# zhangzhousuper/Radish_PT

Hardware: AMD Instinct MI355X
Metric: Mrays/s (higher is better)
Workload: dtype f32

## Files before the change

radish_pt_amd/csrc/device/kernels_wave.h:

```cpp
#pragma once
#include "kernels_pt.h"
#include "wg_trace.h"
#include "ray_cull.h"
#include "kernels_walk.h"

namespace rd {

constexpr int kWfLitCap = 8192;
constexpr int kWfLitShadow = 0x40000000;
constexpr int kMaxWaveDepth = 32;

struct alignas(128) WaveCounter {
    int v;
    int pad[31];
};
#ifndef RD_WF_TICKET_SHARDS
#define RD_WF_TICKET_SHARDS 8
#endif
constexpr int kTicketShards = RD_WF_TICKET_SHARDS;
struct WaveCounters {
    WaveCounter rayCount[kMaxWaveDepth + 2];
    WaveCounter shadowCount[kMaxWaveDepth + 2];
    WaveCounter litCount[kMaxWaveDepth + 2];
    WaveCounter litShadowCount[kMaxWaveDepth + 2];
    WaveCounter traceHead[kMaxWaveDepth + 2];
    WaveCounter shadeHead[kMaxWaveDepth + 2][4];
    WaveCounter traceTicket[kMaxWaveDepth + 2][kTicketShards];
    WaveCounter shadeTicket[kMaxWaveDepth + 2][kTicketShards];
};

struct WaveWorkspace {
    float4 *ro[2];
    float4 *rd[2];
    float4 *thr[2];
    float4 *prevPos[2];
    float4 *accD;
    float4 *accI;
    float4 *nee[2];
    float4 *sht[2];
    uint2 *rng[2];
    int4 *hit;
    int *rayq[2];
    int *shadowq;
    int *litq[2];
    int litCap;
    int *treeOvf;
    int treeOvfDepth;
#ifdef RD_WF_STAMPS
    unsigned long long *stamps;
    int stampWaves;
    int stampStages;
#endif
    WaveCounters *ctr;
};

constexpr unsigned kWfNeeNone = 2u;
RD_DEV float wfNeeTag(int home, unsigned kind) { return __uint_as_float(((unsigned)home << 2) | kind); }
RD_DEV void wfAddNee(const WaveWorkspace &w, float4 n) {
    const unsigned tag = __float_as_uint(n.w), kind = tag & 3u;
    if (kind == kWfNeeNone) return;
    float4 *acc = (kind == 0u ? w.accD : w.accI) + (tag >> 2);
    const float4 a = *acc;
    *acc = make_float4(a.x + n.x, a.y + n.y, a.z + n.z, 0.f);
}

RD_DEV Ray wfSlotRay(const WaveWorkspace &w, int set, int p, bool shadow, float &limit) {
    if (shadow) {
        const float4 x = w.prevPos[set][p], y = w.sht[set][p];
        return shadowRay(mk3(x.x, x.y, x.z), mk3(y.x, y.y, y.z), limit);
    }
    const float4 o = w.ro[set][p], d = w.rd[set][p];
    limit = 3.402823466e+38f;
    return Ray{mk3(o.x, o.y, o.z), mk3(d.x, d.y, d.z)};
}

struct WaveSlotPath {
    const WaveWorkspace &w;
    const int rs, p;
    const int wr, q;
    int home;
    const bool delta;
    bool nullNee = false;
    RD_DEV v3 throughput() {
        const float4 t = w.thr[rs][p];
        home = __float_as_int(t.w);
        return mk3(t.x, t.y, t.z);
    }
    RD_DEV float samplePdf() const { return w.ro[rs][p].w; }
    RD_DEV bool sampleDelta() const { return delta; }
    RD_DEV v3 prevPos() const { const float4 c = w.prevPos[rs][p]; return mk3(c.x, c.y, c.z); }
    RD_DEV void setDirect(v3 v) { w.accD[home] = make_float4(v.x, v.y, v.z, 0.f); }
    RD_DEV void addIndirect(v3 v) { const float4 a = w.accI[home]; w.accI[home] = make_float4(a.x + v.x, a.y + v.y, a.z + v.z, 0.f); }
    RD_DEV Sampler rng(const DScene &s) const { const uint2 r = w.rng[rs][p]; return Sampler{s.sobol, r.x, (int)r.y}; }
    RD_DEV void setNee(v3 c, float nw) {
        w.nee[wr][q] = make_float4(c.x, c.y, c.z, wfNeeTag(home, nw < 0.f ? kWfNeeNone : (nw == 0.f ? 0u : 1u)));
        nullNee = nw < 0.f || (c.x == 0.f && c.y == 0.f && c.z == 0.f);
    }
    RD_DEV void setPrevPos(v3 x) { w.prevPos[wr][q] = make_float4(x.x, x.y, x.z, 0.f); }
    RD_DEV void setRay(const Ray &ray, float pdf, bool deltaSample, v3 throughput, const Sampler &rng) {
        w.ro[wr][q] = make_float4(ray.o.x, ray.o.y, ray.o.z, pdf);
        w.rd[wr][q] = make_float4(ray.d.x, ray.d.y, ray.d.z, deltaSample ? 1.f : 0.f);
        w.thr[wr][q] = make_float4(throughput.x, throughput.y, throughput.z, __int_as_float(home));
        w.rng[wr][q] = make_uint2(rng.scramble, (unsigned)rng.ptr);
    }
};


RD_DEV void waveAppend(bool pred, int item, int *queue, int *count) {
    unsigned long long mask = __ballot(pred);
    if (mask == 0ull) return;
    int leader = __ffsll((long long)mask) - 1;
    int base = 0;
    if ((int)(threadIdx.x & 63u) == leader) base = atomicAdd(count, __popcll(mask));
    base = __shfl(base, leader, 64);
    if (pred) queue[base + __popcll(mask & laneMaskLt())] = item;
}

constexpr int kShadeChunks = 4;
constexpr int kShadePacket = 64 * kShadeChunks;
#ifndef RD_WF_APPEND_CHUNKS
#define RD_WF_APPEND_CHUNKS 16
#endif
static_assert(RD_WF_APPEND_CHUNKS == 4 || RD_WF_APPEND_CHUNKS == 8 || RD_WF_APPEND_CHUNKS == 16, "RD_WF_APPEND_CHUNKS: 4, 8 or 16");
constexpr int kAppendSpan = 64 * RD_WF_APPEND_CHUNKS;

constexpr int kPacket = 128;
RD_DEV int gridWaves() { return int(gridDim.x * (blockDim.x >> 6)); }
RD_DEV int workgroupTicket(WaveCounter *tickets) {
    __shared__ int ticket;
    if (threadIdx.x == 0) {
        const unsigned x = blockIdx.x % (unsigned)kTicketShards;
        ticket = int(x + (unsigned)kTicketShards * (unsigned)atomicAdd(&tickets[x].v, 1));
    }
    __syncthreads();
    return __builtin_amdgcn_readfirstlane(ticket);
}
RD_DEV int logicalWave(int wg) { return __builtin_amdgcn_readfirstlane(int(wg * int(blockDim.x >> 6) + int(threadIdx.x >> 6))); }
RD_DEV int wavePull(int *head, int packet) {
    int base = 0;
    if ((threadIdx.x & 63u) == 0u) base = atomicAdd(head, packet);
    return __shfl(base, 0, 64) + gridWaves() * packet;
}
RD_DEV int tracePull(int *head, int headBase) {
    int base = 0;
    if ((threadIdx.x & 63u) == 0u) base = atomicAdd(head, kPacket);
    return __builtin_amdgcn_readlane(base, 0) + headBase;
}

RD_DEV unsigned subFrameBlocks(const PixelMap &pm, int part, int parts) { return (unsigned)(pm.numBlocks - part + parts - 1) / (unsigned)parts; }
constexpr int kSobolRows = 10000;
template <bool LENS>
RD_DEV void wfRaygen(const DScene &s, const DCamera &cam, const PixelMap &pm, const WaveWorkspace &w, int looper, int samples, int part,
                     int parts, const DLens &lens) {
    unsigned wg;
    const unsigned nLocal = subFrameBlocks(pm, part, parts);
    const unsigned nGroups = nLocal * (unsigned)samples;
    bool wgValid = xcdSwizzle(blockIdx.x, (nGroups + 3u) >> 2, wg);
    unsigned lane = threadIdx.x & 63u;
    unsigned group = wgValid ? wg * 4u + (threadIdx.x >> 6) : 0xffffffffu / 64u;
    const bool inRange = wgValid && group < nGroups;
    const unsigned b = group / nLocal, blockLocal = group - b * nLocal;
    Pix px = mapPixel(pm, inRange ? blockLocal * (unsigned)parts + (unsigned)part : 0xffffffffu / 64u, lane);
    bool valid = px.valid && inRange;
    int p = int(group * 64u + lane);
    bool listed = false;
    if (valid) {
        Sampler rng = makeSeededRandomEngine(int(((unsigned)looper + b) % (unsigned)kSobolRows), px.index, 0, s.sobol);
        Ray ray = cameraSample<LENS>(cam, px.x, px.y, sample4D(rng), lens);
        w.ro[0][p] = make_float4(ray.o.x, ray.o.y, ray.o.z, 0.f);
        w.rd[0][p] = make_float4(ray.d.x, ray.d.y, ray.d.z, 0.f);
        w.accD[p] = make_float4(0.f, 0.f, 0.f, 0.f);
        w.accI[p] = make_float4(0.f, 0.f, 0.f, 0.f);
        w.rng[0][p] = make_uint2(rng.scramble, (unsigned)rng.ptr);
        if (fabs_(ray.d.x) < 1.1e-6f || fabs_(ray.d.y) < 1.1e-6f || fabs_(ray.d.z) < 1.1e-6f) {
            const int at = atomicAdd(&w.ctr->litCount[0].v, 1);
            if (at < w.litCap) {
                w.litq[0][at] = p;
                listed = true;
            }
        }
    }
    if (inRange) w.rayq[0][p] = valid ? (listed ? -2 - p : p) : -1;
    if (blockIdx.x == 0 && threadIdx.x == 0) w.ctr->rayCount[0].v = int(nGroups) * 64;
}
__global__ __launch_bounds__(256) void k_wf_raygen(DScene s, DCamera cam, PixelMap pm, WaveWorkspace w, int looper, int samples, int part,
                                                   int parts) {
    wfRaygen<false>(s, cam, pm, w, looper, samples, part, parts, DLens{});
}
__global__ __launch_bounds__(256) void k_wf_raygen_lens(DScene s, DCamera cam, PixelMap pm, WaveWorkspace w, int looper, int samples,
                                                        int part, int parts, DLens lens) {
    wfRaygen<true>(s, cam, pm, w, looper, samples, part, parts, lens);
}

#ifndef RD_WF_DUTY_SHARE
#define RD_WF_DUTY_SHARE 0
#endif
#ifndef RD_REFILL_MIN
#define RD_REFILL_MIN 16
#endif
#ifndef RD_WF_FINISH_MIN
#define RD_WF_FINISH_MIN 16
#endif
#ifndef RD_WF_SHADOW_FIRST
#define RD_WF_SHADOW_FIRST 0
#endif
constexpr int kWfStampKinds = 6;
#ifdef RD_WF_STAMPS
#define RD_WF_STAMP(kind) do { if (stampAt && (threadIdx.x & 63u) == 0u) stampAt[kind] = wall_clock64(); } while (0)
#define RD_WF_STAMP_DRY() do { if (exhausted && !stampedDry) { stampedDry = true; RD_WF_STAMP(1); if (stampAt && (threadIdx.x & 63u) == 0u) *headDry = 1ull; } } while (0)
#define RD_WF_STAMP_HELD(held) do { if (stampAt && !stampedHeld && *headDry != 0ull) { \
        stampedHeld = true; const int h_ = (held); if ((threadIdx.x & 63u) == 0u) stampAt[4] = 1ull + (unsigned long long)h_; } } while (0)
#else
#define RD_WF_STAMP(kind) ((void)0)
#define RD_WF_STAMP_DRY() ((void)0)
#define RD_WF_STAMP_HELD(held) ((void)0)
#endif
#ifndef RD_WF_COOP_LONE
#define RD_WF_COOP_LONE 1
#endif

#ifndef RD_WF_TRACE_WAVES
#define RD_WF_TRACE_WAVES 7
#endif
#ifndef RD_WF_PAIR_WAVES
#define RD_WF_PAIR_WAVES 1
#endif
#ifndef RD_WF_PAIR_MAX_WAVES
#define RD_WF_PAIR_MAX_WAVES 6
#endif
template <bool COUNT, bool PAIRS = false>
__global__ __launch_bounds__(256) __attribute__((amdgpu_waves_per_eu(PAIRS && !COUNT ? RD_WF_PAIR_WAVES : (!COUNT ? RD_WF_TRACE_WAVES : 1),
                                                                      PAIRS && !COUNT ? RD_WF_PAIR_MAX_WAVES : 8))) void k_wf_trace(DScene s, WaveWorkspace w, int k) {
    WaveCounters *c = w.ctr;
    const int wg = workgroupTicket(c->traceTicket[k]);
#ifdef RD_WF_STAMPS
    unsigned long long *const stampAt = w.stamps ? w.stamps + ((size_t)k * (size_t)w.stampWaves + (size_t)logicalWave(wg)) * kWfStampKinds : nullptr;
    volatile unsigned long long *const headDry = w.stamps ? w.stamps + (size_t)w.stampStages * (size_t)w.stampWaves * kWfStampKinds + k : nullptr;
    bool stampedDry = false, stampedHeld = false;
    RD_WF_STAMP(0);
#endif
    const int nShadow = (k > 0) ? c->shadowCount[k - 1].v : 0;
    const int nRay = c->rayCount[k].v;
    const int total = nShadow + nRay;
    const int *rayq = w.rayq[k & 1];
    const int set = k & 1;
    WalkStats ws{0, 0};
    unsigned nClosest = 0, nAny = 0, nHits = 0;
    const int end = s.bvhSize;
    const int END = end;

    const int nLit = c->litCount[k].v < w.litCap ? c->litCount[k].v : w.litCap;
    const int dutyGroups = RD_WF_DUTY_SHARE ? 0 : (nLit < int(gridDim.x) ? nLit : int(gridDim.x));
    const bool duty = wg < dutyGroups;
    const int headBase = (int(gridDim.x) - dutyGroups) * int(blockDim.x >> 6) * kPacket;
    int resNext = duty ? headBase : (logicalWave(wg) - dutyGroups * int(blockDim.x >> 6)) * kPacket, resEnd = duty ? resNext : resNext + kPacket;
    bool exhausted = resNext >= total;
    if (resEnd > total) resEnd = total;
    RD_WF_STAMP_DRY();

    bool alive = false;
    bool isShadow = false;
    int p = -1;
    RaySlab rs;
    rs.o = rs.d = rs.inv = mk3(0.f);
    rs.cls = 0;
    const NodeRec *nodes = s.nodes[0];
    int ord = 0, cur = kPairNone;
    PairStack sp{0, 0};
    int node = END, pending = -1;
    float tmax = 0.f;
    int hitPrim = -1;
    v2 hitBary = mk2(0.f, 0.f);
    bool occluded = false;

    constexpr int kStackEntries = PAIRS ? 4 * kPairLds * 64 : 1;
    __shared__ union WfTraceLds {
        WgTraceSharedT<256> wg;
        int2 stack[kStackEntries];
    } lds;
    WgTraceSharedT<256> &wgsh = lds.wg;
    int2 *const stk = lds.stack + (PAIRS ? int(threadIdx.x >> 6) * kPairLds * 64 : 0);
    int2 *const ovf = PAIRS ? reinterpret_cast<int2 *>(w.treeOvf) + (size_t)logicalWave(wg) * (size_t)w.treeOvfDepth * 64 : nullptr;
    for (int it = wg; it < nLit; it += int(gridDim.x)) {
        const int e = w.litq[k & 1][it];
        const bool sh = (e & kWfLitShadow) != 0;
        const int pp = e & (kWfLitShadow - 1);
        float lim;
        const Ray ray = wfSlotRay(w, set, pp, sh, lim);
        const RaySlab urs = makeRaySlab(ray);
        if (urs.cls == 0 || end == 0) continue;
        const NodeRec *un = s.nodes[getMTBVHId(-ray.d)];
        const CoopTrace ct = sh ? wgTraceWhole<true, 256>(s, un, urs, lim, wgsh) : wgTraceWhole<false, 256>(s, un, urs, lim, wgsh);
        if (threadIdx.x == 0) {
            if (sh) {
                nAny++;
                if (!ct.found) wfAddNee(w, w.nee[set][pp]);
            } else {
                nClosest++;
                const bool hit = ct.hitPrim != -1;
                if (hit) nHits++;
                w.hit[pp] = make_int4(ct.hitPrim, __float_as_int(hit ? ct.bary.x : 0.f), __float_as_int(hit ? ct.bary.y : 0.f),
                                      hit ? int(s.primClass[ct.hitPrim]) : 0);
            }
            if (COUNT) {
                ws.nodes += ct.nodes;
                ws.tris += ct.tris;
            }
        }
    }
    RD_WF_STAMP(3);
#ifdef RD_WF_STAMPS
    if (stampAt && (threadIdx.x & 63u) == 0u) stampAt[5] = 1ull + (unsigned long long)nLit;
#endif
    if (PAIRS) __syncthreads();
    bool firstRound = true;
    bool fromList = false;
    for (;;) {
        bool doStart = false;
        fromList = false;
        if (firstRound) {
            firstRound = false;
            const int it = wg + (int(threadIdx.x & 63u) * 4 + int(threadIdx.x >> 6)) * int(gridDim.x);
            if (it < nLit) {
                const int e = w.litq[k & 1][it];
                doStart = true;
                fromList = true;
                isShadow = (e & kWfLitShadow) != 0;
                p = e & (kWfLitShadow - 1);
            }
        }
        unsigned long long idle = __ballot(!alive && !doStart && p < 0);
        int nIdle = __popcll(idle);
        if (!exhausted && nIdle >= RD_REFILL_MIN) {
            RD_WF_STAMP_HELD(resEnd - resNext);
            int myRank = __popcll(idle & laneMaskLt());
            int taken = 0;
            while (taken < nIdle && !exhausted) {
                if (resNext == resEnd) {
                    resNext = tracePull(&c->traceHead[k].v, headBase);
                    resEnd = resNext + kPacket;
                    if (resNext >= total) {
                        exhausted = true;
                        break;
                    }
                    if (resEnd > total) resEnd = total;
                }
                int avail = resEnd - resNext;
                int give = (nIdle - taken) < avail ? (nIdle - taken) : avail;
                if (!alive && !doStart && p < 0 && myRank >= taken && myRank < taken + give) {
                    const int item = resNext + (myRank - taken);
                    doStart = true;
#if RD_WF_SHADOW_FIRST
                    isShadow = item < nShadow;
                    p = isShadow ? w.shadowq[item] : rayq[item - nShadow];
#else
                    isShadow = item >= nRay;
                    p = isShadow ? w.shadowq[item - nRay] : rayq[item];
#endif
                }
                resNext += give;
                taken += give;
            }
        }
        RD_WF_STAMP_DRY();
        if (doStart) {
            if (p >= 0) {
                const Ray ray = wfSlotRay(w, set, p, isShadow, tmax);
                if (isShadow) nAny++;
                else nClosest++;
                rs = makeRaySlab(ray);
                pending = -1;
                if (PAIRS) {
                    ord = getMTBVHId(-ray.d);
                    sp = PairStack{0, 0};
                    if (rs.cls == 0 || end == 0) pairStart<COUNT>(s, rs, tmax, cur, pending, ws);
                    else cur = kPairFresh;
                    alive = true;
                } else {
                    nodes = s.nodes[getMTBVHId(-ray.d)];
                    node = 0;
                    alive = node != END;
                }
                hitPrim = -1;
                occluded = false;
                if (fromList && rs.cls != 0 && end != 0) {
                    if (isShadow) nAny--;
                    else nClosest--;
                    alive = false;
                    p = -1;
                }
            }
        }
        unsigned long long am = __ballot(alive);
        if (am == 0ull) {
            if (exhausted) break;
            continue;
        }

        {
            unsigned long long lit = __ballot(PAIRS ? (alive && cur == kPairFresh) : (alive && rs.cls != 0 && node == 0 && pending < 0));
            while (lit) {
                const int L = __ffsll((long long)lit) - 1;
                lit &= lit - 1ull;
                const bool shadowL = readlaneI(isShadow ? 1 : 0, L) != 0;
                const NodeRec *un = PAIRS ? s.nodes[0] + (size_t)readlaneI(ord, L) * (size_t)(end + 1) : readlanePtr(nodes, L);
                const RaySlab ur = readlaneRay(rs, L);
                const float lim = readlaneF(tmax, L);
                CoopTrace ct = shadowL ? coopTraceWhole<true>(s, un, ur, lim) : coopTraceWhole<false>(s, un, ur, lim);
                if (int(threadIdx.x & 63u) == L) {
                    hitPrim = ct.hitPrim;
                    hitBary = ct.bary;
                    tmax = ct.tmax;
                    occluded = ct.found;
                    node = END;
                    cur = kPairNone;
                    alive = false;
                    if (COUNT) {
                        ws.nodes += ct.nodes;
                        ws.tris += ct.tris;
                    }
                }
            }
        }
        if (PAIRS) {
            bool busy = alive && pending < 0;
            const int nStart = __popcll(__ballot(busy));
            if (nStart > 0) {
                const int minWalk = (nStart * (RD_LEAF_DEN - RD_LEAF_NUM) + RD_LEAF_DEN - 1) / RD_LEAF_DEN;
                const int lane = int(threadIdx.x & 63u);
                do {
                    pairPopOne<COUNT>(stk, lane, ovf, tmax, busy, cur, sp, pending, ws);
                    if (busy && cur >= 0) {
                        pairStep<COUNT>(s.pairs, stk, lane, ovf, rs, tmax, ord, cur, sp, pending, ws);
                        busy = pending < 0 && (cur >= 0 || sp.sp > 0);
                    }
                } while (__popcll(__ballot(busy)) >= (minWalk > 1 ? minWalk : 1));
                alive = alive && (pending >= 0 || cur >= 0 || sp.sp > 0);
            }
        } else
        {
            bool walking = alive && pending < 0;
            const int nStart = __popcll(__ballot(walking));
#if RD_WF_COOP_LONE
            if (nStart == 1) {
                const int L = __ffsll((long long)__ballot(walking)) - 1;
                CoopResult cr = coopWalk(readlanePtr(nodes, L), readlaneI(node, L), end, readlaneRay(rs, L), readlaneF(tmax, L), RD_COOP_WINDOWS);
                if (int(threadIdx.x & 63u) == L) {
                    node = cr.node;
                    pending = cr.pending;
                    if (COUNT) ws.nodes += cr.visited;
                    alive = (node != end) || pending >= 0;
                }
            } else
#endif
            if (nStart > 0) {
                const int minWalk = (nStart * (RD_LEAF_DEN - RD_LEAF_NUM) + RD_LEAF_DEN - 1) / RD_LEAF_DEN;
                do {
                    if (walking) {
                        if (COUNT) ws.nodes++;
                        float4 lo = nodes[node].lo_prim;
                        float4 hi = nodes[node].hi_next;
                        float boundDist;
                        bool boundHit = aabbFast(lo, hi, rs, boundDist);
                        if (boundHit && boundDist < tmax) {
                            pending = __float_as_int(lo.w);
                            node++;
                        } else {
                            node = __float_as_int(hi.w);
                        }
                        walking = pending < 0 && node != END;
                        alive = (node != END) || pending >= 0;
                    }
                } while (__popcll(__ballot(walking)) >= (minWalk > 1 ? minWalk : 1));
            }
        }
        if (alive && pending >= 0) {
            TriVerts t = loadTri(s.tris, pending);
            float dist;
            v2 bary;
            if (COUNT) ws.tris++;
            bool hit = intersectTriangle(rs, t.a, t.b, t.c, bary, dist);
            if (hit && dist < tmax) {
                if (isShadow) {
                    occluded = true;
                    node = END;
                    cur = kPairNone;
                    sp = PairStack{0, 0};
                } else {
                    hitPrim = pending;
                    tmax = dist;
                    hitBary = bary;
                }
            }
            pending = -1;
            alive = PAIRS ? (cur >= 0 || sp.sp > 0) : (node != END);
        }
        const unsigned long long doneM = __ballot(!alive && p >= 0);
        if (doneM != 0ull && __popcll(doneM) * 64 >= (__popcll(doneM) + __popcll(__ballot(alive))) * RD_WF_FINISH_MIN)
        if (!alive && p >= 0) {
            if (isShadow) {
                if (!occluded) wfAddNee(w, w.nee[set][p]);
            } else {
                bool hit = hitPrim != -1;
                if (hit) nHits++;
                w.hit[p] = make_int4(hitPrim, __float_as_int(hit ? hitBary.x : 0.f), __float_as_int(hit ? hitBary.y : 0.f),
                                     hit ? int(s.primClass[hitPrim]) : 0);
            }
            p = -1;
        }
    }
    RD_WF_STAMP(2);
    if (COUNT) flushCounters(s.counters, nClosest, nAny, nHits, ws);
}

struct WfSlotWork {
    const WaveWorkspace &w;
    int p;

    RD_DEV bool find(long long chunk, int slot) {
        const int e = w.rayq[0][chunk * 64 + slot];
        p = e <= -2 ? -2 - e : e;
        return e != -1;
    }
    RD_DEV Ray ray(float &tmax) const { return wfSlotRay(w, 0, p, false, tmax); }
    RD_DEV void store(const DScene &s, const RaySlab &, int hitPrim, v2 hitBary, float, bool) const {
        const bool hit = hitPrim != -1;
        w.hit[p] = make_int4(hitPrim, __float_as_int(hit ? hitBary.x : 0.f), __float_as_int(hit ? hitBary.y : 0.f),
                             hit ? int(s.primClass[hitPrim]) : 0);
    }
};
#ifndef RD_WF_PRIMARY_WAVES
#define RD_WF_PRIMARY_WAVES 1
#endif
template <bool COUNT>
__global__ __launch_bounds__(256, COUNT ? 1 : RD_WF_PRIMARY_WAVES) void k_wf_trace_primary(DScene s, WaveWorkspace w, int nGroups, int budget) {
    __shared__ WgTraceSharedT<256> wgsh;
    const int nLit = w.ctr->litCount[0].v < w.litCap ? w.ctr->litCount[0].v : w.litCap;
    WalkStats ws{0, 0};
    unsigned nClosest = 0, nHits = 0;
    for (int it = int(blockIdx.x); it < nLit; it += int(gridDim.x)) {
        const int pp = w.litq[0][it];
        float lim;
        const Ray ray = wfSlotRay(w, 0, pp, false, lim);
        const RaySlab urs = makeRaySlab(ray);
        if (!raySetAside(urs.cls) || s.bvhSize == 0) continue;
        const CoopTrace ct = wgTraceWhole<false, 256>(s, s.nodes[getMTBVHId(-ray.d)], urs, lim, wgsh);
        if (threadIdx.x == 0) {
            nClosest++;
            const bool hit = ct.hitPrim != -1;
            if (hit) nHits++;
            w.hit[pp] = make_int4(ct.hitPrim, __float_as_int(hit ? ct.bary.x : 0.f), __float_as_int(hit ? ct.bary.y : 0.f),
                                  hit ? int(s.primClass[ct.hitPrim]) : 0);
            if (COUNT) {
                ws.nodes += ct.nodes;
                ws.tris += ct.tris;
            }
        }
    }
    if (COUNT && threadIdx.x < 64u) flushCounters(s.counters, nClosest, 0u, nHits, ws);
    const int group = int(blockIdx.x) * 4 + int(threadIdx.x >> 6);
    if (group >= nGroups) return;
    const bool listed = w.rayq[0][(size_t)group * 64 + (threadIdx.x & 63u)] <= -2;
    WfSlotWork work{w, -1};
    walkPacket<COUNT, true>(s, group, listed, budget, work);
}

constexpr int kSortChunks = 16;
constexpr int kSortPacket = 64 * kSortChunks;
#ifndef RD_WF_SHADE_WAVES
#define RD_WF_SHADE_WAVES 1
#endif
#ifndef RD_WF_CULL_LAST
#define RD_WF_CULL_LAST 1
#endif
#ifndef RD_WF_SKIP_NULL_NEE
#define RD_WF_SKIP_NULL_NEE 1
#endif
__global__ __launch_bounds__(256, RD_WF_SHADE_WAVES) void k_wf_shade(DScene s, WaveWorkspace w, int k, int maxDepth, int sorted,
                                                                     const float4 *__restrict__ emitBox, int walkAll) {
    __shared__ int sSorted[4][kSortPacket];
    WaveCounters *c = w.ctr;
    const bool cullLast = RD_WF_CULL_LAST && !walkAll && k + 1 == maxDepth && !hasEnvMap(s);
    const bool skipNull = RD_WF_SKIP_NULL_NEE && !walkAll;
    float4 boxLo = make_float4(0.f, 0.f, 0.f, 0.f), boxHi = boxLo;
    if (cullLast) {
        boxLo = emitBox[0];
        boxHi = emitBox[1];
    }
    const int wg = workgroupTicket(c->shadeTicket[k]);
    const int lane = int(threadIdx.x & 63u);
    int *mySorted = sSorted[threadIdx.x >> 6];
    {
        const int q = 0;
        const int n = c->rayCount[k].v;
        const int *hitq = w.rayq[k & 1];
        int pendShadows = 0, pendRays = 0;
        int packet = kShadePacket;
        if (sorted) {
            const int perWave = n / (2 * gridWaves());
            packet = ((perWave + kShadePacket - 1) / kShadePacket) * kShadePacket;
            packet = packet < kShadePacket ? kShadePacket : (packet > kSortPacket ? kSortPacket : packet);
        }
        int packetEnd = 0;
        for (int base = logicalWave(wg) * packet, sub = 0, fresh = 1;;) {
            if (sub == packet) {
                base = wavePull(&c->shadeHead[k][q].v, packet);
                sub = 0;
                fresh = 1;
            }
            if (base + sub >= n) break;
            if (sorted && fresh) {
                fresh = 0;
                packetEnd = (n - base) < packet ? (n - base) : packet;
                int pp[kSortChunks], cls[kSortChunks];
#pragma unroll
                for (int j = 0; j < kSortChunks; j++) {
                    const int i = base + j * 64 + lane;
                    pp[j] = (j * 64 + lane < packetEnd) ? hitq[i] : -1;
                    if (pp[j] <= -2) pp[j] = -2 - pp[j];
                }
#pragma unroll
                for (int j = 0; j < kSortChunks; j++) {
                    cls[j] = (pp[j] >= 0) ? w.hit[pp[j]].w : 0;
                }
                int at = 0;
#pragma unroll
                for (int qq = 0; qq < 4; qq++) {
#pragma unroll
                    for (int j = 0; j < kSortChunks; j++) {
                        const bool in = (j * 64 + lane < packetEnd) && cls[j] == qq;
                        const unsigned long long m = __ballot(in);
                        if (in) mySorted[at + __popcll(m & laneMaskLt())] = pp[j];
                        at += __popcll(m);
                    }
                }
                __builtin_amdgcn_wave_barrier();
            }
            int item = base + sub + lane;
            const int subNow = sub;
            sub += 64;
            bool active = sorted ? (subNow + lane < packetEnd) : (item < n);
            bool emitShadow = false, emitRay = false, litShadow = false, litRay = false, rayFirst = false;
            int p = -1;
            const int q = base + subNow + lane;
            if (active) {
                p = sorted ? mySorted[subNow + lane] : hitq[item];
                if (p <= -2) p = -2 - p;
                active = p >= 0;
            }
            if (active) {
                const int4 h = w.hit[p];
                const float4 rdw = w.rd[k & 1][p];
                WaveSlotPath st{w, k & 1, p, (k + 1) & 1, q, p, rdw.w != 0.f};
                const PathStepResult r = pathStep(s, k, maxDepth, h.x, mk2(__int_as_float(h.y), __int_as_float(h.z)), mk3(rdw.x, rdw.y, rdw.z), st);
                if (r.shadow && !(skipNull && st.nullNee)) {
                    w.sht[(k + 1) & 1][q] = make_float4(r.shadowTo.x, r.shadowTo.y, r.shadowTo.z, 0.f);
                    emitShadow = true;
                    const v3 dl = r.shadowTo - r.shadowFrom;
                    const float l2 = dot(dl, dl) * 1.21e-12f;
                    litShadow = dl.x * dl.x < l2 || dl.y * dl.y < l2 || dl.z * dl.z < l2;
                }
                if (r.extension && !(cullLast && !mayReachEmitters(boxLo, boxHi, r.ray.o, r.ray.d))) {
                    emitRay = true;
                    litRay = fabs_(r.ray.d.x) < 1.1e-6f || fabs_(r.ray.d.y) < 1.1e-6f || fabs_(r.ray.d.z) < 1.1e-6f;
                }
            }
            if (__ballot(litShadow || litRay) != 0ull) {
                int *lq = w.litq[(k + 1) & 1];
                int *lc = &c->litCount[k + 1].v;
                for (int kind = 0; kind < 2; kind++) {
                    const bool pred = kind == 0 ? litShadow : litRay;
                    const unsigned long long m = __ballot(pred);
                    if (m == 0ull) continue;
                    int at = 0;
                    if (lane == 0) at = atomicAdd(lc, __popcll(m));
                    at = __shfl(at, 0, 64) + __popcll(m & laneMaskLt());
                    if (kind == 0) {
                        const int listed = __popcll(__ballot(pred && at < w.litCap));
                        if (lane == 0 && listed > 0) atomicAdd(&c->litShadowCount[k].v, listed);
                    }
                    if (pred && at < w.litCap) {
                        lq[at] = kind == 0 ? (q | kWfLitShadow) : q;
                        if (kind == 0) emitShadow = false;
                        else rayFirst = true;
                    }
                }
            }
            mySorted[subNow + lane] = (emitShadow ? 1 : 0) | (emitRay ? 2 : 0) | (rayFirst ? 4 : 0);
            pendShadows += __popcll(__ballot(emitShadow));
            pendRays += __popcll(__ballot(emitRay));
            if ((sub & (kAppendSpan - 1)) == 0 || sub == packet || base + sub >= n) {
                int atS = 0, atR = 0;
                if (lane == 0) {
                    if (pendShadows > 0) atS = atomicAdd(&c->shadowCount[k].v, pendShadows);
                    if (pendRays > 0) atR = atomicAdd(&c->rayCount[k + 1].v, pendRays);
                }
                atS = __builtin_amdgcn_readfirstlane(atS);
                atR = __builtin_amdgcn_readfirstlane(atR);
                int *nextq = w.rayq[(k + 1) & 1];
                for (int o = subNow & ~(kAppendSpan - 1); o < sub; o += 64) {
                    const int f = mySorted[o + lane], qq = base + o + lane;
                    const unsigned long long mS = __ballot((f & 1) != 0), mR = __ballot((f & 2) != 0);
                    if (f & 1) w.shadowq[atS + __popcll(mS & laneMaskLt())] = qq;
                    if (f & 2) nextq[atR + __popcll(mR & laneMaskLt())] = (f & 4) ? -2 - qq : qq;
                    atS += __popcll(mS);
                    atR += __popcll(mR);
                }
                pendShadows = pendRays = 0;
            }
        }
    }
}

RD_DEV v3 foldRunningMean(v3 mean, float4 acc, int iter) {
    return (mean * float(iter) + finishSample(mk3(acc.x, acc.y, acc.z))) / float(iter + 1);
}
__global__ __launch_bounds__(256) void k_wf_finish(PixelMap pm, WaveWorkspace w, int iter, int samples, float *__restrict__ directIllum,
                                                   float *__restrict__ indirectIllum, int part, int parts) {
    unsigned wg;
    const unsigned nLocal = subFrameBlocks(pm, part, parts);
    bool wgValid = xcdSwizzle(blockIdx.x, (nLocal + 3u) >> 2, wg);
    unsigned lane = threadIdx.x & 63u;
    unsigned blockLocal = wgValid ? wg * 4u + (threadIdx.x >> 6) : 0xffffffffu / 64u;
    const bool inRange = wgValid && blockLocal < nLocal;
    Pix px = mapPixel(pm, inRange ? blockLocal * (unsigned)parts + (unsigned)part : 0xffffffffu / 64u, lane);
    if (!(px.valid && inRange)) return;
    v3 direct = load3(directIllum, px.out), indirect = load3(indirectIllum, px.out);
    for (int b = 0; b < samples; b++) {
        const int p = int(((unsigned)b * nLocal + blockLocal) * 64u + lane);
        direct = foldRunningMean(direct, w.accD[p], iter + b);
        indirect = foldRunningMean(indirect, w.accI[p], iter + b);
    }
    store3(directIllum, px.out, direct);
    store3(indirectIllum, px.out, indirect);
}

}
```

Baseline: 3476.

## Defer shade queue appends and batch packet pull with counter atomics

Restructures the shade kernel so that each packet's shadow and ray counts are reserved once per packet. The reservation uses a single multi-lane atomic that also pulls the next packet from the work head. The queue writes for a packet are deferred until after the next packet has been binned, using double-buffered LDS rows, so the atomic latency overlaps with the next packet's loads. This doubles the per-wave LDS footprint and changes the append granularity from spans to whole packets, which may reduce occupancy.

```diff
diff --git a/radish_pt_amd/csrc/device/kernels_wave.h b/radish_pt_amd/csrc/device/kernels_wave.h
--- a/radish_pt_amd/csrc/device/kernels_wave.h
+++ b/radish_pt_amd/csrc/device/kernels_wave.h
@@ -576,9 +576,14 @@
 #ifndef RD_WF_SKIP_NULL_NEE
 #define RD_WF_SKIP_NULL_NEE 1
 #endif
+#ifndef RD_WF_DEFER_APPENDS
+#define RD_WF_DEFER_APPENDS 1
+#endif
+static_assert(RD_WF_DEFER_APPENDS >= 0 && RD_WF_DEFER_APPENDS <= 2, "RD_WF_DEFER_APPENDS: 0, 1 or 2");
+constexpr int kShadeRows = RD_WF_DEFER_APPENDS == 1 ? 2 : 1;
 __global__ __launch_bounds__(256, RD_WF_SHADE_WAVES) void k_wf_shade(DScene s, WaveWorkspace w, int k, int maxDepth, int sorted,
                                                                      const float4 *__restrict__ emitBox, int walkAll) {
-    __shared__ int sSorted[4][kSortPacket];
+    __shared__ int sSorted[4][kShadeRows][kSortPacket];
     WaveCounters *c = w.ctr;
     const bool cullLast = RD_WF_CULL_LAST && !walkAll && k + 1 == maxDepth && !hasEnvMap(s);
     const bool skipNull = RD_WF_SKIP_NULL_NEE && !walkAll;
@@ -589,127 +594,170 @@
     }
     const int wg = workgroupTicket(c->shadeTicket[k]);
     const int lane = int(threadIdx.x & 63u);
-    int *mySorted = sSorted[threadIdx.x >> 6];
-    {
-        const int q = 0;
-        const int n = c->rayCount[k].v;
-        const int *hitq = w.rayq[k & 1];
+    int *myRows = sSorted[threadIdx.x >> 6][0];
+    const int n = c->rayCount[k].v;
+    const int *hitq = w.rayq[k & 1];
+    int *nextq = w.rayq[(k + 1) & 1];
+    int *head = &c->shadeHead[k][0].v;
+    int packet = kShadePacket;
+    if (sorted) {
+        const int perWave = n / (2 * gridWaves());
+        packet = ((perWave + kShadePacket - 1) / kShadePacket) * kShadePacket;
+        packet = packet < kShadePacket ? kShadePacket : (packet > kSortPacket ? kSortPacket : packet);
+    }
+    auto binPacket = [&](int *row, int base, int packetEnd) __attribute__((always_inline)) {
+        int pp[kSortChunks], cls[kSortChunks];
+#pragma unroll
+        for (int j = 0; j < kSortChunks; j++) {
+            const int i = base + j * 64 + lane;
+            pp[j] = (j * 64 + lane < packetEnd) ? hitq[i] : -1;
+            if (pp[j] <= -2) pp[j] = -2 - pp[j];
+        }
+#pragma unroll
+        for (int j = 0; j < kSortChunks; j++) {
+            cls[j] = (pp[j] >= 0) ? w.hit[pp[j]].w : 0;
+        }
+        int at = 0;
+#pragma unroll
+        for (int qq = 0; qq < 4; qq++) {
+#pragma unroll
+            for (int j = 0; j < kSortChunks; j++) {
+                const bool in = (j * 64 + lane < packetEnd) && cls[j] == qq;
+                const unsigned long long m = __ballot(in);
+                if (in) row[at + __popcll(m & laneMaskLt())] = pp[j];
+                at += __popcll(m);
+            }
+        }
+        __builtin_amdgcn_wave_barrier();
+    };
+    auto shadeChunk = [&](int *row, int base, int subNow, int packetEnd, int &pendShadows, int &pendRays) __attribute__((always_inline)) {
+        const int item = base + subNow + lane;
+        bool active = sorted ? (subNow + lane < packetEnd) : (item < n);
+        bool emitShadow = false, emitRay = false, litShadow = false, litRay = false, rayFirst = false;
+        int p = -1;
+        const int q = base + subNow + lane;
+        if (active) {
+            p = sorted ? row[subNow + lane] : hitq[item];
+            if (p <= -2) p = -2 - p;
+            active = p >= 0;
+        }
+        if (active) {
+            const int4 h = w.hit[p];
+            const float4 rdw = w.rd[k & 1][p];
+            WaveSlotPath st{w, k & 1, p, (k + 1) & 1, q, p, rdw.w != 0.f};
+            const PathStepResult r = pathStep(s, k, maxDepth, h.x, mk2(__int_as_float(h.y), __int_as_float(h.z)), mk3(rdw.x, rdw.y, rdw.z), st);
+            if (r.shadow && !(skipNull && st.nullNee)) {
+                w.sht[(k + 1) & 1][q] = make_float4(r.shadowTo.x, r.shadowTo.y, r.shadowTo.z, 0.f);
+                emitShadow = true;
+                const v3 dl = r.shadowTo - r.shadowFrom;
+                const float l2 = dot(dl, dl) * 1.21e-12f;
+                litShadow = dl.x * dl.x < l2 || dl.y * dl.y < l2 || dl.z * dl.z < l2;
+            }
+            if (r.extension && !(cullLast && !mayReachEmitters(boxLo, boxHi, r.ray.o, r.ray.d))) {
+                emitRay = true;
+                litRay = fabs_(r.ray.d.x) < 1.1e-6f || fabs_(r.ray.d.y) < 1.1e-6f || fabs_(r.ray.d.z) < 1.1e-6f;
+            }
+        }
+        if (__ballot(litShadow || litRay) != 0ull) {
+            int *lq = w.litq[(k + 1) & 1];
+            int *lc = &c->litCount[k + 1].v;
+            for (int kind = 0; kind < 2; kind++) {
+                const bool pred = kind == 0 ? litShadow : litRay;
+                const unsigned long long m = __ballot(pred);
+                if (m == 0ull) continue;
+                int at = 0;
+                if (lane == 0) at = atomicAdd(lc, __popcll(m));
+                at = __shfl(at, 0, 64) + __popcll(m & laneMaskLt());
+                if (kind == 0) {
+                    const int listed = __popcll(__ballot(pred && at < w.litCap));
+                    if (lane == 0 && listed > 0) atomicAdd(&c->litShadowCount[k].v, listed);
+                }
+                if (pred && at < w.litCap) {
+                    lq[at] = kind == 0 ? (q | kWfLitShadow) : q;
+                    if (kind == 0) emitShadow = false;
+                    else rayFirst = true;
+                }
+            }
+        }
+        row[subNow + lane] = (emitShadow ? 1 : 0) | (emitRay ? 2 : 0) | (rayFirst ? 4 : 0);
+        pendShadows += __popcll(__ballot(emitShadow));
+        pendRays += __popcll(__ballot(emitRay));
+    };
+    auto writeEntries = [&](const int *row, int base, int from, int to, int atS, int atR) __attribute__((always_inline)) {
+        for (int o = from; o < to; o += 64) {
+            const int f = row[o + lane], qq = base + o + lane;
+            const unsigned long long mS = __ballot((f & 1) != 0), mR = __ballot((f & 2) != 0);
+            if (f & 1) w.shadowq[atS + __popcll(mS & laneMaskLt())] = qq;
+            if (f & 2) nextq[atR + __popcll(mR & laneMaskLt())] = (f & 4) ? -2 - qq : qq;
+            atS += __popcll(mS);
+            atR += __popcll(mR);
+        }
+    };
+#if RD_WF_DEFER_APPENDS
+    auto addToCounters = [&](int pull, int shadows, int rays) __attribute__((always_inline)) {
+        int *ctr = lane == 0 ? head : (lane == 1 ? &c->shadowCount[k].v : &c->rayCount[k + 1].v);
+        const int v = lane == 0 ? pull : (lane == 1 ? shadows : rays);
+        int got = 0;
+        if (lane < 3 && v > 0) got = atomicAdd(ctr, v);
+        return got;
+    };
+    int base = logicalWave(wg) * packet;
+    if (base >= n) return;
+    int cur = 0;
+    int heldBase = 0, heldExt = 0;
+    int held = 0;
+    for (;;) {
+        int *row = myRows + cur * kSortPacket;
+        const int packetEnd = (n - base) < packet ? (n - base) : packet;
+        if (sorted) binPacket(row, base, packetEnd);
+        if (heldExt > 0)
+            writeEntries(myRows + (cur ^ 1) * kSortPacket, heldBase, 0, heldExt, __builtin_amdgcn_readlane(held, 1), __builtin_amdgcn_readlane(held, 2));
         int pendShadows = 0, pendRays = 0;
-        int packet = kShadePacket;
-        if (sorted) {
-            const int perWave = n / (2 * gridWaves());
-            packet = ((perWave + kShadePacket - 1) / kShadePacket) * kShadePacket;
-            packet = packet < kShadePacket ? kShadePacket : (packet > kSortPacket ? kSortPacket : packet);
-        }
-        int packetEnd = 0;
-        for (int base = logicalWave(wg) * packet, sub = 0, fresh = 1;;) {
-            if (sub == packet) {
-                base = wavePull(&c->shadeHead[k][q].v, packet);
-                sub = 0;
-                fresh = 1;
-            }
-            if (base + sub >= n) break;
-            if (sorted && fresh) {
-                fresh = 0;
-                packetEnd = (n - base) < packet ? (n - base) : packet;
-                int pp[kSortChunks], cls[kSortChunks];
-#pragma unroll
-                for (int j = 0; j < kSortChunks; j++) {
-                    const int i = base + j * 64 + lane;
-                    pp[j] = (j * 64 + lane < packetEnd) ? hitq[i] : -1;
-                    if (pp[j] <= -2) pp[j] = -2 - pp[j];
-                }
-#pragma unroll
-                for (int j = 0; j < kSortChunks; j++) {
-                    cls[j] = (pp[j] >= 0) ? w.hit[pp[j]].w : 0;
-                }
-                int at = 0;
-#pragma unroll
-                for (int qq = 0; qq < 4; qq++) {
-#pragma unroll
-                    for (int j = 0; j < kSortChunks; j++) {
-                        const bool in = (j * 64 + lane < packetEnd) && cls[j] == qq;
-                        const unsigned long long m = __ballot(in);
-                        if (in) mySorted[at + __popcll(m & laneMaskLt())] = pp[j];
-                        at += __popcll(m);
-                    }
-                }
-                __builtin_amdgcn_wave_barrier();
-            }
-            int item = base + sub + lane;
-            const int subNow = sub;
-            sub += 64;
-            bool active = sorted ? (subNow + lane < packetEnd) : (item < n);
-            bool emitShadow = false, emitRay = false, litShadow = false, litRay = false, rayFirst = false;
-            int p = -1;
-            const int q = base + subNow + lane;
-            if (active) {
-                p = sorted ? mySorted[subNow + lane] : hitq[item];
-                if (p <= -2) p = -2 - p;
-                active = p >= 0;
-            }
-            if (active) {
-                const int4 h = w.hit[p];
-                const float4 rdw = w.rd[k & 1][p];
-                WaveSlotPath st{w, k & 1, p, (k + 1) & 1, q, p, rdw.w != 0.f};
-                const PathStepResult r = pathStep(s, k, maxDepth, h.x, mk2(__int_as_float(h.y), __int_as_float(h.z)), mk3(rdw.x, rdw.y, rdw.z), st);
-                if (r.shadow && !(skipNull && st.nullNee)) {
-                    w.sht[(k + 1) & 1][q] = make_float4(r.shadowTo.x, r.shadowTo.y, r.shadowTo.z, 0.f);
-                    emitShadow = true;
-                    const v3 dl = r.shadowTo - r.shadowFrom;
-                    const float l2 = dot(dl, dl) * 1.21e-12f;
-                    litShadow = dl.x * dl.x < l2 || dl.y * dl.y < l2 || dl.z * dl.z < l2;
-                }
-                if (r.extension && !(cullLast && !mayReachEmitters(boxLo, boxHi, r.ray.o, r.ray.d))) {
-                    emitRay = true;
-                    litRay = fabs_(r.ray.d.x) < 1.1e-6f || fabs_(r.ray.d.y) < 1.1e-6f || fabs_(r.ray.d.z) < 1.1e-6f;
-                }
-            }
-            if (__ballot(litShadow || litRay) != 0ull) {
-                int *lq = w.litq[(k + 1) & 1];
-                int *lc = &c->litCount[k + 1].v;
-                for (int kind = 0; kind < 2; kind++) {
-                    const bool pred = kind == 0 ? litShadow : litRay;
-                    const unsigned long long m = __ballot(pred);
-                    if (m == 0ull) continue;
-                    int at = 0;
-                    if (lane == 0) at = atomicAdd(lc, __popcll(m));
-                    at = __shfl(at, 0, 64) + __popcll(m & laneMaskLt());
-                    if (kind == 0) {
-                        const int listed = __popcll(__ballot(pred && at < w.litCap));
-                        if (lane == 0 && listed > 0) atomicAdd(&c->litShadowCount[k].v, listed);
-                    }
-                    if (pred && at < w.litCap) {
-                        lq[at] = kind == 0 ? (q | kWfLitShadow) : q;
-                        if (kind == 0) emitShadow = false;
-                        else rayFirst = true;
-                    }
-                }
-            }
-            mySorted[subNow + lane] = (emitShadow ? 1 : 0) | (emitRay ? 2 : 0) | (rayFirst ? 4 : 0);
-            pendShadows += __popcll(__ballot(emitShadow));
-            pendRays += __popcll(__ballot(emitRay));
-            if ((sub & (kAppendSpan - 1)) == 0 || sub == packet || base + sub >= n) {
-                int atS = 0, atR = 0;
-                if (lane == 0) {
-                    if (pendShadows > 0) atS = atomicAdd(&c->shadowCount[k].v, pendShadows);
-                    if (pendRays > 0) atR = atomicAdd(&c->rayCount[k + 1].v, pendRays);
-                }
-                atS = __builtin_amdgcn_readfirstlane(atS);
-                atR = __builtin_amdgcn_readfirstlane(atR);
-                int *nextq = w.rayq[(k + 1) & 1];
-                for (int o = subNow & ~(kAppendSpan - 1); o < sub; o += 64) {
-                    const int f = mySorted[o + lane], qq = base + o + lane;
-                    const unsigned long long mS = __ballot((f & 1) != 0), mR = __ballot((f & 2) != 0);
-                    if (f & 1) w.shadowq[atS + __popcll(mS & laneMaskLt())] = qq;
-                    if (f & 2) nextq[atR + __popcll(mR & laneMaskLt())] = (f & 4) ? -2 - qq : qq;
-                    atS += __popcll(mS);
-                    atR += __popcll(mR);
-                }
-                pendShadows = pendRays = 0;
-            }
-        }
-    }
+        for (int sub = 0; sub < packetEnd; sub += 64) shadeChunk(row, base, sub, packetEnd, pendShadows, pendRays);
+        const bool full = packetEnd == packet;
+        heldBase = base;
+        heldExt = (packetEnd + 63) & ~63;
+        held = addToCounters(full ? packet : 0, pendShadows, pendRays);
+        if (!full) break;
+        base = __builtin_amdgcn_readlane(held, 0) + gridWaves() * packet;
+        if (base >= n) break;
+#if RD_WF_DEFER_APPENDS == 2
+        writeEntries(row, heldBase, 0, heldExt, __builtin_amdgcn_readlane(held, 1), __builtin_amdgcn_readlane(held, 2));
+        heldExt = 0;
+#else
+        cur ^= 1;
+#endif
+    }
+    writeEntries(myRows + cur * kSortPacket, heldBase, 0, heldExt, __builtin_amdgcn_readlane(held, 1), __builtin_amdgcn_readlane(held, 2));
+#else
+    int pendShadows = 0, pendRays = 0;
+    int packetEnd = 0;
+    for (int base = logicalWave(wg) * packet, sub = 0, fresh = 1;;) {
+        if (sub == packet) {
+            base = wavePull(head, packet);
+            sub = 0;
+            fresh = 1;
+        }
+        if (base + sub >= n) break;
+        if (sorted && fresh) {
+            fresh = 0;
+            packetEnd = (n - base) < packet ? (n - base) : packet;
+            binPacket(myRows, base, packetEnd);
+        }
+        const int subNow = sub;
+        sub += 64;
+        shadeChunk(myRows, base, subNow, packetEnd, pendShadows, pendRays);
+        if ((sub & (kAppendSpan - 1)) == 0 || sub == packet || base + sub >= n) {
+            int atS = 0, atR = 0;
+            if (lane == 0) {
+                if (pendShadows > 0) atS = atomicAdd(&c->shadowCount[k].v, pendShadows);
+                if (pendRays > 0) atR = atomicAdd(&c->rayCount[k + 1].v, pendRays);
+            }
+            writeEntries(myRows, base, subNow & ~(kAppendSpan - 1), sub, __builtin_amdgcn_readfirstlane(atS), __builtin_amdgcn_readfirstlane(atR));
+            pendShadows = pendRays = 0;
+        }
+    }
+#endif
 }
 
 RD_DEV v3 foldRunningMean(v3 mean, float4 acc, int iter) {
```

Result: no change. 3507 (median of 6 runs) (+0.9%).
